# zhu-xlab/tomosar2height

Hardware: AMD Instinct MI355X
Metric: training tiles/sec (Berlin crop, cloud-only) (higher is better)
Workload: dtype f32; 1 GPU; BASELINE.json configs[1]: Berlin cloud-only, fp32 per-point GEMMs, train_step(tile) per tile, 4 tiles coalesced per forward/backward (Trainer default), N=131072 points/tile, R=256, ALTO depth 5, 512x512 target, optimize_every=64; points_per_tile=131072, optimize_every=64, train_batch=1, coalesce_tiles=4, optimizer=t2h FlatAdamW (one kernel over the flat bucket), parallelism=dp1, rccl_ranks=0, channels_last=True, point_distribution=70 % in 160 buildings + 30 % uniform, grid_convs=conv_bx3.hip: fp32 products from 3 fp16 MFMAs (2-way split, block scales), library_fallbacks=0, hip_graph=False

## Files before the change

tomosar2height_amd/csrc/conv_bx3.hip:

```cpp
#include <stdlib.h>
#include "t2h_common.h"
#include "gemm_args.h"
#include "gemm_tile.h"

namespace t2h {
namespace {

using bf16x8 = __attribute__((ext_vector_type(8))) __bf16;
using f16x8 = __attribute__((ext_vector_type(8))) _Float16;
using f16x2 = __attribute__((ext_vector_type(2))) _Float16;
using bf16x2 = __attribute__((ext_vector_type(2))) __bf16;
using f32x2 = __attribute__((ext_vector_type(2))) float;
using s16x4 = __attribute__((ext_vector_type(4))) short;
using s16x8 = __attribute__((ext_vector_type(8))) short;
typedef __attribute__((address_space(3))) void lds_void;
typedef const __attribute__((address_space(1))) void glb_void;
typedef __attribute__((address_space(3))) s16x4 lds_s16x4;

#ifndef T2H_BX3_BDIRECT
#define T2H_BX3_BDIRECT 1
#endif
constexpr int NT = 256;
constexpr int TW = 32;
constexpr int CC = 32;
// ... 502 lines not shown
                old.x = mk.x > 0.f ? old.x : 0.f; old.y = mk.y > 0.f ? old.y : 0.f;
                old.z = mk.z > 0.f ? old.z : 0.f; old.w = mk.w > 0.f ? old.w : 0.f;
            }
            v.x += bv.x; v.y += bv.y; v.z += bv.z; v.w += bv.w;
            if (UPM == 1) {
                float4 *dst = reinterpret_cast<float4 *>(p.y + q);
                if (accum) { v.x += old.x; v.y += old.y; v.z += old.z; v.w += old.w; }
                if (p.addend) { v.x += mk.x; v.y += mk.y; v.z += mk.z; v.w += mk.w; }
                *dst = v;
                continue;
            }
            if (p.mask) {
                v.x = mk.x > 0.f ? v.x : 0.f; v.y = mk.y > 0.f ? v.y : 0.f;
                v.z = mk.z > 0.f ? v.z : 0.f; v.w = mk.w > 0.f ? v.w : 0.f;
            }
            if (relu) { v.x = relu1(v.x); v.y = relu1(v.y); v.z = relu1(v.z); v.w = relu1(v.w); }
            float4 *dst = reinterpret_cast<float4 *>(ybase + q * p.ldy + col);
            if (accum) { v.x += old.x; v.y += old.y; v.z += old.z; v.w += old.w; }
            *dst = v;
        }
    }
  }
}

struct WgradArgs {
    const float *dy;
    const float *x;
    float *slab;
    float *colslab;
    int H, W, Cin, Cout;
    int n_units, units_per_split;
    int ldx;
    int lddy;
};

template <int COT, int NPL, bool UP = false, int GT = 0>
__global__ __launch_bounds__(NT, 2) void bx3_wgrad_kernel(WgradArgs p) {
    static_assert(!(UP && GT), "UP and GT are different forms");
    constexpr int NTAPS = GT ? GT : (UP ? 4 : 9);
    constexpr int WPC = 4 / COT;
    constexpr int TMAX = (NTAPS + WPC - 1) / WPC;
    constexpr int YS = COT == 1 ? 64 : 64 * COT + 64;
    constexpr int XS = 64;
    constexpr int YPLANE = 32 * YS, XHP = GT ? GT * TW : (UP ? 4 * TW : 3 * (TW + 2)), XPLANE = XHP * XS;
    constexpr int LDS_WORK = NPL * YPLANE + NPL * XPLANE;
    constexpr int LDS_BYTES = LDS_WORK >= 4 * 32 * 36 * 4 ? LDS_WORK : 4 * 32 * 36 * 4;
    constexpr bool H2 = NPL == 2;
    __shared__ __attribute__((aligned(1024))) unsigned char lds[LDS_BYTES + (H2 ? 64 : 0)];
    unsigned char *yimg = lds, *ximg = lds + NPL * YPLANE;
    float *slots = reinterpret_cast<float *>(lds + LDS_BYTES);

    const int tid = threadIdx.x, lane = tid & 63, wave = tid >> 6;
    const int split = GT ? blockIdx.z : blockIdx.x, ci0 = GT ? 0 : blockIdx.y * CC, co0 = (GT ? blockIdx.x : blockIdx.z) * (32 * COT);
    const int u_beg = split * p.units_per_split, u_end = min(p.n_units, u_beg + p.units_per_split);
    const int segs = p.W / TW;

    const int cot = wave / WPC, sub = wave % WPC;
    const int tap_lo = (NTAPS * sub + WPC - 1) / WPC, tap_hi = (NTAPS * (sub + 1) + WPC - 1) / WPC;

    constexpr int XF4 = XHP * 8, XPER = (XF4 + NT - 1) / NT;
    constexpr int YPER = COT;
    float4 xr[XPER], yr[YPER];
    auto load_unit = [&](int u) {
        const int xs = u % segs, row = u / segs;
        const int y = row & (p.H - 1), x0 = xs * TW;
#pragma unroll
        for (int f = 0; f < XPER; ++f) {
            const int idx = tid + f * NT;
            const int px = idx >> 3, c4 = idx & 7;
            const int hy = px / (TW + 2), hx = px - hy * (TW + 2);
            const int gy = y + hy - 1, gx = x0 + hx - 1;
            float4 v = make_float4(0.f, 0.f, 0.f, 0.f);
            if (GT) {
                if (idx < XF4) v = *reinterpret_cast<const float4 *>(p.x + ((size_t)u * TW + (px % TW)) * p.ldx + (px / TW) * 32 + c4 * 4);
            } else if (UP) {
                v = *reinterpret_cast<const float4 *>(p.x + ((size_t)(2 * row + (px >> 6)) * (2 * p.W) + 2 * x0 + (px & 63)) * p.ldx + ci0 + c4 * 4);
            } else if (idx < XF4 && (unsigned)gy < (unsigned)p.H && (unsigned)gx < (unsigned)p.W)
                v = *reinterpret_cast<const float4 *>(p.x + ((size_t)(row + hy - 1) * p.W + gx) * p.ldx + ci0 + c4 * 4);
            xr[f] = v;
        }
#pragma unroll
        for (int f = 0; f < YPER; ++f) {
            const int idx = tid + f * NT;
            const int px = idx / (8 * COT), c4 = idx % (8 * COT);
            yr[f] = *reinterpret_cast<const float4 *>(p.dy + ((size_t)row * p.W + x0 + px) * (GT ? p.lddy : p.Cout) + co0 + c4 * 4);
        }
    };
    float4 csum = make_float4(0.f, 0.f, 0.f, 0.f);
    const bool do_colsum = p.colslab != nullptr && (UP ? blockIdx.z == 0 : blockIdx.y == 0);
    int s_run = E_UNSET, ex_cur = 0, ey_cur = 0;
    auto publish_unit_max = [&](int parity) {
        float mx = 0.f, my = 0.f;
#pragma unroll
        for (int f = 0; f < XPER; ++f) mx = abs4max(mx, xr[f]);
#pragma unroll
        for (int f = 0; f < YPER; ++f) my = abs4max(my, yr[f]);
        mx = wave_max(mx);
        my = wave_max(my);
        if (lane == 0) { slots[(parity * 4 + wave) * 2] = mx; slots[(parity * 4 + wave) * 2 + 1] = my; }
    };
    auto store_unit = [&]() {
#pragma unroll
        for (int f = 0; f < XPER; ++f) {
            const int idx = tid + f * NT;
            if (idx < XF4) {
                const int c4 = idx & 7;
                int px = idx >> 3;
                if (UP) {
                    px = ((px >> 6) * 2 + (px & 1)) * TW + ((px & 63) >> 1);
                    if (do_colsum) { csum.x += xr[f].x; csum.y += xr[f].y; csum.z += xr[f].z; csum.w += xr[f].w; }
                }
                unsigned a1, a2, a3, b1, b2, b3;
                unsigned char *d = ximg + px * XS + c4 * 8;
                if (H2) {
                    split2h(xr[f].x, xr[f].y, ex_cur, a1, a2);
                    split2h(xr[f].z, xr[f].w, ex_cur, b1, b2);
                    *reinterpret_cast<uint2 *>(d) = make_uint2(a1, b1);
                    *reinterpret_cast<uint2 *>(d + XPLANE) = make_uint2(a2, b2);
                    continue;
                }
                split3(xr[f].x, xr[f].y, a1, a2, a3);
                split3(xr[f].z, xr[f].w, b1, b2, b3);
                *reinterpret_cast<uint2 *>(d) = make_uint2(a1, b1);
                if (NPL == 3) {
                    *reinterpret_cast<uint2 *>(d + XPLANE) = make_uint2(a2, b2);
                    *reinterpret_cast<uint2 *>(d + 2 * XPLANE) = make_uint2(a3, b3);
                }
            }
        }
#pragma unroll
        for (int f = 0; f < YPER; ++f) {
            const int idx = tid + f * NT;
            const int px = idx / (8 * COT), c4 = idx % (8 * COT);
            unsigned a1, a2, a3, b1, b2, b3;
            unsigned char *d = yimg + px * YS + c4 * 8;
            if (!UP && do_colsum) { csum.x += yr[f].x; csum.y += yr[f].y; csum.z += yr[f].z; csum.w += yr[f].w; }
            if (H2) {
                split2h(yr[f].x, yr[f].y, ey_cur, a1, a2);
                split2h(yr[f].z, yr[f].w, ey_cur, b1, b2);
                *reinterpret_cast<uint2 *>(d) = make_uint2(a1, b1);
                *reinterpret_cast<uint2 *>(d + YPLANE) = make_uint2(a2, b2);
                continue;
            }
            split3(yr[f].x, yr[f].y, a1, a2, a3);
            split3(yr[f].z, yr[f].w, b1, b2, b3);
            *reinterpret_cast<uint2 *>(d) = make_uint2(a1, b1);
            if (NPL == 3) {
                *reinterpret_cast<uint2 *>(d + YPLANE) = make_uint2(a2, b2);
                *reinterpret_cast<uint2 *>(d + 2 * YPLANE) = make_uint2(a3, b3);
            }
        }
    };

    f32x16 acc[TMAX];
#pragma unroll
    for (int t = 0; t < TMAX; ++t)
#pragma unroll
        for (int z = 0; z < 16; ++z) acc[t][z] = 0.0f;

    const int g = lane >> 4, gi = lane & 15, gq = gi >> 2, gp = gi & 3;
    const int kpix = 8 * (g >> 1) + gq;
    const int choff = (16 * (g & 1) + 4 * gp) * 2;
    auto tr8 = [&](const unsigned char *a, int row_stride) -> bf16x8 {
        const s16x4 lo = __builtin_amdgcn_ds_read_tr16_b64_v4i16((lds_s16x4 *)(a));
        const s16x4 hi = __builtin_amdgcn_ds_read_tr16_b64_v4i16((lds_s16x4 *)(a + 4 * row_stride));
        const s16x8 v = __builtin_shufflevector(lo, hi, 0, 1, 2, 3, 4, 5, 6, 7);
        return *reinterpret_cast<const bf16x8 *>(&v);
    };

    if (u_beg < u_end) load_unit(u_beg);
    if (H2) {
        if (u_beg < u_end) publish_unit_max(u_beg & 1);
        __syncthreads();
    }
    for (int u = u_beg; u < u_end; ++u) {
        if (H2) {
            const float *sl = slots + (u & 1) * 8;
            const int ex_nat = block_exponent(__float_as_uint(fmaxf(fmaxf(sl[0], sl[2]), fmaxf(sl[4], sl[6]))));
            const int ey_nat = block_exponent(__float_as_uint(fmaxf(fmaxf(sl[1], sl[3]), fmaxf(sl[5], sl[7]))));
            if (ex_nat != E_UNSET && ey_nat != E_UNSET && ex_nat + ey_nat < s_run) {
                if (s_run != E_UNSET) {
#pragma unroll
                    for (int t = 0; t < TMAX; ++t)
#pragma unroll
                        for (int z = 0; z < 16; ++z) acc[t][z] = ldexpf(acc[t][z], ex_nat + ey_nat - s_run);
                }
                s_run = ex_nat + ey_nat;
            }
            ex_cur = ex_nat == E_UNSET ? 0 : ex_nat;
            ey_cur = ey_nat == E_UNSET ? 0 : (s_run == E_UNSET ? ey_nat : min(s_run - ex_cur, ey_nat));
        }
        store_unit();
        if (u + 1 < u_end) load_unit(u + 1);
        __syncthreads();
#pragma unroll
        for (int s = 0; s < 2; ++s) {
            bf16x8 af[NPL];
            const unsigned char *ya = yimg + (16 * s + kpix) * YS + cot * 64 + choff;
#pragma unroll
            for (int pl = 0; pl < NPL; ++pl) af[pl] = tr8(ya + pl * YPLANE, YS);
#pragma unroll
            for (int t = 0; t < TMAX; ++t) {
                const int tap = tap_lo + t;
                if (tap < tap_hi) {
                    const int ky = tap / 3, kx = tap - 3 * ky;
                    const unsigned char *xa = ximg + ((UP || GT) ? tap * TW + 16 * s + kpix : ky * (TW + 2) + 16 * s + kpix + kx) * XS + choff;
                    bf16x8 bfr[NPL];
#pragma unroll
                    for (int pl = 0; pl < NPL; ++pl) bfr[pl] = tr8(xa + pl * XPLANE, XS);
                    constexpr int ia[6] = {2, 0, 1, 1, 0, 0}, ib[6] = {0, 2, 1, 0, 1, 0};
                    if (H2) {
#pragma unroll
                        for (int e = 3; e < 6; ++e)
                            acc[t] = __builtin_amdgcn_mfma_f32_32x32x16_f16(*reinterpret_cast<const f16x8 *>(&af[ia[e]]),
                                                                            *reinterpret_cast<const f16x8 *>(&bfr[ib[e]]), acc[t], 0, 0, 0);
                    } else {
#pragma unroll
                        for (int e = (NPL == 3 ? 0 : 5); e < 6; ++e)
                            acc[t] = __builtin_amdgcn_mfma_f32_32x32x16_bf16(af[ia[e]], bfr[ib[e]], acc[t], 0, 0, 0);
                    }
                }
            }
        }
        if (H2 && u + 1 < u_end) publish_unit_max((u + 1) & 1);
        __syncthreads();
    }

    if (do_colsum) {
        float4 *red = reinterpret_cast<float4 *>(lds);
        red[tid] = csum;
        __syncthreads();
        constexpr int CG = UP ? 8 : 8 * COT;
        if (tid < CG) {
            float4 tsum = red[tid];
            for (int j = tid + CG; j < NT; j += CG) { tsum.x += red[j].x; tsum.y += red[j].y; tsum.z += red[j].z; tsum.w += red[j].w; }
            if (UP) *reinterpret_cast<float4 *>(p.colslab + (size_t)split * p.Cin + ci0 + tid * 4) = tsum;
            else *reinterpret_cast<float4 *>(p.colslab + (size_t)split * p.Cout + co0 + tid * 4) = tsum;
        }
        __syncthreads();
    }

    float *patch = reinterpret_cast<float *>(lds) + wave * (32 * 36);
    const int er = lane >> 3, ec = (lane & 7) * 4, r = lane & 31, h = lane >> 5;
    float *sbase = p.slab + (size_t)split * p.Cout * NTAPS * p.Cin;
#pragma unroll
    for (int t = 0; t < TMAX; ++t) {
        const int tap = tap_lo + t;
        if (tap < tap_hi) {
#pragma unroll
            for (int z = 0; z < 16; ++z)
                patch[((z & 3) + 8 * (z >> 2) + 4 * h) * 36 + r] = H2 ? ldexpf(acc[t][z], s_run == E_UNSET ? 0 : -s_run) : acc[t][z];
#pragma unroll
            for (int pass = 0; pass < 4; ++pass) {
                const float4 v = *reinterpret_cast<const float4 *>(patch + (pass * 8 + er) * 36 + ec);
                const int co = co0 + cot * 32 + pass * 8 + er;
                *reinterpret_cast<float4 *>(sbase + ((size_t)co * NTAPS + tap) * p.Cin + ci0 + ec) = v;
            }
        }
    }
}

bool al16(const void *q) { return (uintptr_t)q % 16 == 0; }
bool pow2(int v) { return v > 0 && (v & (v - 1)) == 0; }

int check_bx3(const char *what, int B, int H, int W, int Cin, int Cout) {
    if (B < 1 || !pow2(H) || !pow2(W) || H < 4 || W < TW || H > 32768 || W > 32768 || Cin < 32 || Cout < 32 || Cin % 32 || Cout % 32)
        return fail(T2H_ERR_ARG, "%s: needs power-of-two H >= 4, W >= 32 and Cin, Cout multiples of 32 (B=%d H=%d W=%d %d->%d)", what, B,
                    H, W, Cin, Cout);
    if ((long long)B * H * W > (1LL << 30)) return fail(T2H_ERR_ARG, "%s: more than 2^30 pixels", what);
    return T2H_OK;
}

struct RowsPlan { bool tall; int bn, splits, chunks_per_split; long long tiles; };
RowsPlan bx3_rows_plan(int B, int H, int W, int Kc, int Nc, int ntap = 9, int upm = 0) {
    RowsPlan r{};
    r.bn = Nc % 128 == 0 ? 128 : (Nc % 64 == 0 ? 64 : 32);
    if (upm) {
        r.tall = false;
        const long long row_tiles = (long long)B * (H / 4) * (W / TW);
        if (upm == 1) while (r.bn > 32 && row_tiles * (Nc / r.bn) < 192) r.bn >>= 1;
        r.tiles = row_tiles * (Nc / r.bn);
        r.splits = 1;
        const int nchunk_u = Kc / 64;
        static const long long target_u = 512;
        if (upm == 2 && r.tiles < target_u / 2) {
            long long want = (target_u + r.tiles - 1) / r.tiles;
            if (want > nchunk_u) want = nchunk_u;
            if (want > 32) want = 32;
            r.splits = (int)(want < 1 ? 1 : want);
// ... 88 lines not shown
            else BX3_LAUNCH(4, 32, 4, 1, 32, 9);
        }
    } else if (ntap == 1 && upm == 0 && npl == 2 && a.Kc == 64 && r.splits == 1 && a.Nc / r.bn >= 8 && persist_n_enabled()) {
        const long long row_tiles = (long long)a.B * (a.H / 4) * (a.W / TW);
        const int pbn = r.bn == 128 ? 64 : r.bn;
        const int ntn = a.Nc / pbn;
        static const long long persist_wgs = getenv("T2H_BX3_PERSIST_WGS") ? atoll(getenv("T2H_BX3_PERSIST_WGS")) : 2048;
        static const long long min_groups = getenv("T2H_BX3_PERSIST_MIN_GROUPS") ? atoll(getenv("T2H_BX3_PERSIST_MIN_GROUPS")) : 4;
        long long groups = persist_wgs / (row_tiles > 0 ? row_tiles : 1);
        if (groups < min_groups) groups = min_groups;
        if (groups < 1) groups = 1;
        if (groups > ntn) groups = ntn;
        a.ntn_per_wg = (int)((ntn + groups - 1) / groups);
        groups = (ntn + a.ntn_per_wg - 1) / a.ntn_per_wg;
        const long long pgrid = row_tiles * groups;
        if (pbn == 64) { hipLaunchKernelGGL((bx3_rows_kernel<4, 64, 4, 1, 64, 2, 1, 0, true>), dim3((unsigned)pgrid), dim3(NT), 0, s, a); note_kernel("bx3_rows_kernel<4,64,4,1,64,2,1,0,true>"); }
        else { hipLaunchKernelGGL((bx3_rows_kernel<4, 32, 4, 1, 64, 2, 1, 0, true>), dim3((unsigned)pgrid), dim3(NT), 0, s, a); note_kernel("bx3_rows_kernel<4,32,4,1,64,2,1,0,true>"); }
    } else {
        if (r.tall) {
            if (r.bn == 128) BX3_LAUNCH(8, 128, 2, 2, 32, 1);
            else if (r.bn == 64) BX3_LAUNCH(8, 64, 4, 1, 32, 1);
            else BX3_LAUNCH(8, 32, 4, 1, 32, 1);
        } else {
            if (r.bn == 128) BX3_LAUNCH(4, 128, 2, 2, 64, 1);
            else if (r.bn == 64) BX3_LAUNCH(4, 64, 4, 1, 64, 1);
            else BX3_LAUNCH(4, 32, 4, 1, 64, 1);
        }
    }
    if (int rc = check_launch(what)) return rc;
    if (r.splits > 1) return launch_reduce_rows_epilogue(static_cast<const float *>(ws), r.splits, M * a.Nc, M, a.Nc, e, s);
    return T2H_OK;
}

struct WgradPlan { int cot, splits, units_per_split, n_units; };
WgradPlan bx3_wgrad_plan(int B, int H, int W, int Cin, int Cout) {
    WgradPlan p{};
    p.cot = Cout % 128 == 0 ? 4 : (Cout % 64 == 0 ? 2 : 1);
    p.n_units = B * H * (W / TW);
    const long long groups = (long long)(Cin / CC) * (Cout / (32 * p.cot));
    static const long long forced = getenv("T2H_BX3_WGRAD_WGS") ? atoll(getenv("T2H_BX3_WGRAD_WGS")) : 0;
    const long long target = forced > 0 ? forced : ((long long)H * W <= 128 * 128 ? 256 : 512);
    long long splits = target / groups;
    if (splits < 1) splits = 1;
    if (splits > p.n_units) splits = p.n_units;
    p.units_per_split = (int)((p.n_units + splits - 1) / splits);
    p.splits = (p.n_units + p.units_per_split - 1) / p.units_per_split;
    return p;
}

}
}

using namespace t2h;

T2H_API int t2h_conv3x3_bx3_supported(int B, int H, int W, int Cin, int Cout) {
    return B >= 1 && pow2(H) && pow2(W) && H >= 4 && W >= TW && H <= 32768 && W <= 32768 && Cin >= 32 && Cout >= 32 && Cin % 32 == 0 &&
           Cout % 32 == 0 && (long long)B * H * W <= (1LL << 30);
}

T2H_API size_t t2h_conv3x3_bx3_weights_bytes(int Cin, int Cout) {
    if (Cin < 32 || Cout < 32 || Cin % 32 || Cout % 32) return 0;
    return (size_t)Cout * 9 * Cin * 6;
}

T2H_API int t2h_conv3x3_bx3_prepare(const float *w, int Cin, int Cout, int transposed, void *wf, t2h_stream_t stream) {
    if (!w || !wf) return fail(T2H_ERR_ARG, "conv3x3_bx3_prepare: null pointer");
    if (Cin < 32 || Cout < 32 || Cin % 32 || Cout % 32 || !al16(wf))
        return fail(T2H_ERR_ARG, "conv3x3_bx3_prepare: Cin=%d, Cout=%d must be multiples of 32, wf 16-byte aligned", Cin, Cout);
    const int Kc = transposed ? Cout : Cin, Nc = transposed ? Cin : Cout;
    const long long total = (long long)(Kc / 16) * 9 * (Nc / 32) * 64;
    const unsigned blocks = (unsigned)((total + 255) / 256);
    if (transposed) hipLaunchKernelGGL(bx3_prepare_kernel<true>, dim3(blocks), dim3(256), 0, as_stream(stream), w, Cin, Cout, static_cast<unsigned *>(wf));
// ... 33 lines not shown
    if (!al16(dy) || !al16(wf_t) || !al16(dx) || (mask && !al16(mask))) return fail(T2H_ERR_ARG, "conv3x3_bx3_dgrad: pointers must be 16-byte aligned");
    RowsArgs a{};
    a.x = dy; a.wf = static_cast<const unsigned *>(wf_t); a.bias = nullptr; a.mask = mask; a.y = dx;
    a.B = B; a.H = H; a.W = W; a.Kc = Cout; a.Nc = Cin; a.ldx = Cout; a.ldy = Cin; a.ldm = Cin;
    a.flags = (flags & T2H_ACCUM) ? F_ACCUM : 0;
    a.wscale = f16_trailer(wf_t, (size_t)Cout * 9 * Cin * 4);
    return launch_rows(a, npl_of(flags), workspace, workspace_bytes, as_stream(stream), "conv3x3_bx3_dgrad");
}

T2H_API int t2h_conv3x3_bx3_dgrad_rank1_supported(int B, int H, int W, int Cin, int Cout) {
    if (!t2h_conv3x3_bx3_supported(B, H, W, Cin, Cout)) return 0;
    return bx3_rows_plan(B, H, W, Cout, Cin).splits == 1;
}

T2H_API int t2h_conv3x3_bx3_dgrad_rank1(const float *dy, const void *wf_t, float *dx, const float *mask, const float *g, const float *w1,
                                        int B, int H, int W, int Cin, int Cout, int flags, t2h_stream_t stream) {
    if (!dy || !wf_t || !dx || !g || !w1) return fail(T2H_ERR_ARG, "conv3x3_bx3_dgrad_rank1: null pointer");
    if (int rc = check_bx3("conv3x3_bx3_dgrad_rank1", B, H, W, Cin, Cout)) return rc;
    if (!t2h_conv3x3_bx3_dgrad_rank1_supported(B, H, W, Cin, Cout))
        return fail(T2H_ERR_ARG, "conv3x3_bx3_dgrad_rank1: this shape splits its reduction (use t2h_conv3x3_bx3_dgrad with T2H_ACCUM)");
    if (flags & T2H_ACCUM) return fail(T2H_ERR_ARG, "conv3x3_bx3_dgrad_rank1: the rank-1 term takes the place of the accumulated values");
    if (!al16(dy) || !al16(wf_t) || !al16(dx) || (mask && !al16(mask)) || !al16(w1))
        return fail(T2H_ERR_ARG, "conv3x3_bx3_dgrad_rank1: pointers must be 16-byte aligned");
    RowsArgs a{};
    a.x = dy; a.wf = static_cast<const unsigned *>(wf_t); a.bias = nullptr; a.mask = mask; a.y = dx;
    a.B = B; a.H = H; a.W = W; a.Kc = Cout; a.Nc = Cin; a.ldx = Cout; a.ldy = Cin; a.ldm = Cin;
    a.flags = 0; a.r1_g = g; a.r1_w = w1;
    a.wscale = f16_trailer(wf_t, (size_t)Cout * 9 * Cin * 4);
    return launch_rows(a, npl_of(flags), nullptr, 0, as_stream(stream), "conv3x3_bx3_dgrad_rank1");
}

T2H_API size_t t2h_conv3x3_bx3_wgrad_workspace_bytes(int B, int H, int W, int Cin, int Cout) {
    if (!t2h_conv3x3_bx3_supported(B, H, W, Cin, Cout)) return 0;
    WgradPlan p = bx3_wgrad_plan(B, H, W, Cin, Cout);
    return (size_t)p.splits * ((size_t)Cout * 9 * Cin + Cout) * sizeof(float);
}

T2H_API int t2h_conv3x3_bx3_wgrad(const float *dy, const float *x, float *dw, float *db, int B, int H, int W, int Cin, int Cout,
                                  int flags, void *workspace, size_t workspace_bytes, t2h_stream_t stream) {
    if (!dy || !x || !dw) return fail(T2H_ERR_ARG, "conv3x3_bx3_wgrad: null pointer");
    if (int rc = check_bx3("conv3x3_bx3_wgrad", B, H, W, Cin, Cout)) return rc;
    if (!al16(dy) || !al16(x)) return fail(T2H_ERR_ARG, "conv3x3_bx3_wgrad: pointers must be 16-byte aligned");
    const size_t need = t2h_conv3x3_bx3_wgrad_workspace_bytes(B, H, W, Cin, Cout);
    if (!workspace || workspace_bytes < need || !al16(workspace))
        return fail(T2H_ERR_WORKSPACE, "conv3x3_bx3_wgrad: workspace %zu < %zu bytes", workspace_bytes, need);
    hipStream_t s = as_stream(stream);
    WgradPlan p = bx3_wgrad_plan(B, H, W, Cin, Cout);
    const int Ncols = 9 * Cin;
    float *slab = static_cast<float *>(workspace);
    float *colslab = slab + (size_t)p.splits * Cout * Ncols;
    WgradArgs a{};
    a.dy = dy; a.x = x; a.slab = slab; a.colslab = db ? colslab : nullptr;
    a.H = H; a.W = W; a.Cin = Cin; a.Cout = Cout; a.n_units = p.n_units; a.units_per_split = p.units_per_split; a.ldx = Cin;
    dim3 grid(p.splits, Cin / CC, Cout / (32 * p.cot));
    if (grid.y > 65535 || grid.z > 65535) return fail(T2H_ERR_ARG, "conv3x3_bx3_wgrad: too many channel chunks");
    if (flags & T2H_F16X2) {
        if (p.cot == 4) { hipLaunchKernelGGL((bx3_wgrad_kernel<4, 2>), grid, dim3(NT), 0, s, a); note_kernel("bx3_wgrad_kernel<4,2,false,0>"); }
        else if (p.cot == 2) { hipLaunchKernelGGL((bx3_wgrad_kernel<2, 2>), grid, dim3(NT), 0, s, a); note_kernel("bx3_wgrad_kernel<2,2,false,0>"); }
        else { hipLaunchKernelGGL((bx3_wgrad_kernel<1, 2>), grid, dim3(NT), 0, s, a); note_kernel("bx3_wgrad_kernel<1,2,false,0>"); }
    } else if (flags & T2H_BF16) {
        if (p.cot == 4) { hipLaunchKernelGGL((bx3_wgrad_kernel<4, 1>), grid, dim3(NT), 0, s, a); note_kernel("bx3_wgrad_kernel<4,1,false,0>"); }
        else if (p.cot == 2) { hipLaunchKernelGGL((bx3_wgrad_kernel<2, 1>), grid, dim3(NT), 0, s, a); note_kernel("bx3_wgrad_kernel<2,1,false,0>"); }
        else { hipLaunchKernelGGL((bx3_wgrad_kernel<1, 1>), grid, dim3(NT), 0, s, a); note_kernel("bx3_wgrad_kernel<1,1,false,0>"); }
    } else {
        if (p.cot == 4) { hipLaunchKernelGGL((bx3_wgrad_kernel<4, 3>), grid, dim3(NT), 0, s, a); note_kernel("bx3_wgrad_kernel<4,3,false,0>"); }
        else if (p.cot == 2) { hipLaunchKernelGGL((bx3_wgrad_kernel<2, 3>), grid, dim3(NT), 0, s, a); note_kernel("bx3_wgrad_kernel<2,3,false,0>"); }
        else { hipLaunchKernelGGL((bx3_wgrad_kernel<1, 3>), grid, dim3(NT), 0, s, a); note_kernel("bx3_wgrad_kernel<1,3,false,0>"); }
    }
    if (int rc = check_launch("conv3x3_bx3_wgrad")) return rc;
    return launch_reduce_slabs(slab, p.splits, (long long)Cout * Ncols, Cout, Ncols, Ncols, (flags & T2H_ACCUM) ? 1 : 0, dw, colslab, db, s,
                               0, 0, (flags & T2H_DEFER_REDUCE) != 0);
}

T2H_API int t2h_gemm_bx3_supported(int64_t M, int K, int N) {
    return M >= 128 && M % 128 == 0 && M <= (1LL << 30) && K >= 64 && K % 64 == 0 && N >= 32 && N % 32 == 0;
}

T2H_API size_t t2h_gemm_bx3_weights_bytes(int K, int N) {
    if (K < 16 || N < 32 || K % 16 || N % 32) return 0;
    return (size_t)K * N * 6;
}

T2H_API int t2h_gemm_bx3_prepare(const float *w, int ldw, int K, int N, int w_is_kn, void *wf, t2h_stream_t stream) {
    if (!w || !wf) return fail(T2H_ERR_ARG, "gemm_bx3_prepare: null pointer");
    if (K < 16 || N < 32 || K % 16 || N % 32 || !al16(wf) || ldw < (w_is_kn ? N : K))
        return fail(T2H_ERR_ARG, "gemm_bx3_prepare: K=%d must be a multiple of 16, N=%d of 32, ldw=%d at least the row length", K, N, ldw);
    const long long total = (long long)(K / 16) * (N / 32) * 64;
// ... 32 lines not shown
    if (splits > units) splits = units;
    if (splits < 1) splits = 1;
    const long long per = (units + splits - 1) / splits;
    return (int)((units + per - 1) / per);
}

T2H_API int t2h_gemm_bx3_wgrad_supported(int64_t M, int K, int N) {
    return M >= TW && M % TW == 0 && M <= (1LL << 30) && (K == 64 || K == 128 || K == 256) && N >= 64 && N % 64 == 0;
}

T2H_API size_t t2h_gemm_bx3_wgrad_workspace_bytes(int64_t M, int K, int N) {
    if (!t2h_gemm_bx3_wgrad_supported(M, K, N)) return 0;
    return (size_t)gemm_wgrad_splits(M, N) * ((size_t)N * K + N) * sizeof(float);
}

T2H_API int t2h_gemm_bx3_wgrad(const float *dy, int lddy, const float *x, int ldx, int64_t M, int K, int N, float *dw, float *db, int flags,
                               void *workspace, size_t workspace_bytes, t2h_stream_t stream) {
    if (!dy || !x || !dw) return fail(T2H_ERR_ARG, "gemm_bx3_wgrad: null pointer");
    if (!t2h_gemm_bx3_wgrad_supported(M, K, N))
        return fail(T2H_ERR_ARG, "gemm_bx3_wgrad: needs M %% 32 == 0, K in {64, 128, 256}, N %% 64 == 0 (M=%lld K=%d N=%d)", (long long)M, K, N);
    if (lddy < N || ldx < K || lddy % 4 || ldx % 4 || !al16(dy) || !al16(x))
        return fail(T2H_ERR_ARG, "gemm_bx3_wgrad: rows must be 16-byte aligned and at least N / K floats long");
    if (!(flags & T2H_F16X2)) return fail(T2H_ERR_ARG, "gemm_bx3_wgrad: only the fp16 two-way split (T2H_F16X2) is built");
    const size_t need = t2h_gemm_bx3_wgrad_workspace_bytes(M, K, N);
    if (!workspace || workspace_bytes < need || !al16(workspace))
        return fail(T2H_ERR_WORKSPACE, "gemm_bx3_wgrad: workspace %zu < %zu bytes", workspace_bytes, need);
    hipStream_t s = as_stream(stream);
    const int splits = gemm_wgrad_splits(M, N);
    float *slab = static_cast<float *>(workspace);
    float *colslab = slab + (size_t)splits * N * K;
    WgradArgs a{};
    a.dy = dy; a.x = x; a.slab = slab; a.colslab = db ? colslab : nullptr;
    a.H = (int)(M / TW); a.W = TW; a.Cin = 32; a.Cout = N; a.n_units = (int)(M / TW);
    a.units_per_split = (a.n_units + splits - 1) / splits; a.ldx = ldx; a.lddy = lddy;
    const dim3 grid(N / 64, 1, splits);
    if (grid.z > 65535) return fail(T2H_ERR_ARG, "gemm_bx3_wgrad: too many splits");
    if (K == 64) { hipLaunchKernelGGL((bx3_wgrad_kernel<2, 2, false, 2>), grid, dim3(NT), 0, s, a); note_kernel("bx3_wgrad_kernel<2,2,false,2>"); }
    else if (K == 128) { hipLaunchKernelGGL((bx3_wgrad_kernel<2, 2, false, 4>), grid, dim3(NT), 0, s, a); note_kernel("bx3_wgrad_kernel<2,2,false,4>"); }
    else { hipLaunchKernelGGL((bx3_wgrad_kernel<2, 2, false, 8>), grid, dim3(NT), 0, s, a); note_kernel("bx3_wgrad_kernel<2,2,false,8>"); }
    if (int rc = check_launch("gemm_bx3_wgrad")) return rc;
    return launch_reduce_slabs(slab, splits, (long long)N * K, N, K, K, (flags & T2H_ACCUM) ? 1 : 0, dw, colslab, db, s, 0, 0,
                               (flags & T2H_DEFER_REDUCE) != 0);
}

static int check_up_bx3(const char *what, int B, int H, int W, int Cin, int Cout) {
    if (B < 1 || !pow2(H) || !pow2(W) || H > 16384 || W > 16384 || (long long)B * H * W % 128 != 0 || (long long)B * H * W > (1LL << 28) ||
        Cin < 64 || Cout < 64 || Cin % 64 || Cout % 64)
        return fail(T2H_ERR_ARG, "%s: needs power-of-two H, W with B H W %% 128 == 0 and Cin, Cout multiples of 64 (B=%d H=%d W=%d %d->%d)",
                    what, B, H, W, Cin, Cout);
    return T2H_OK;
}
static int ilog2i(int v) { int l = 0; while ((1 << l) < v) ++l; return l; }

T2H_API int t2h_upconv2x2_bx3_supported(int B, int H, int W, int Cin, int Cout) {
    return B >= 1 && pow2(H) && pow2(W) && H <= 16384 && W <= 16384 && (long long)B * H * W % 128 == 0 && (long long)B * H * W <= (1LL << 28) &&
           Cin >= 64 && Cout >= 64 && Cin % 64 == 0 && Cout % 64 == 0;
}

T2H_API int t2h_upconv2x2_bx3_fwd(const float *x, const void *wf, const float *bias, const float *addend, float *y, int B, int H, int W,
                                  int Cin, int Cout, int flags, t2h_stream_t stream) {
    if (!x || !wf || !y) return fail(T2H_ERR_ARG, "upconv2x2_bx3_fwd: null pointer");
    if (int rc = check_up_bx3("upconv2x2_bx3_fwd", B, H, W, Cin, Cout)) return rc;
    if (!al16(x) || !al16(wf) || !al16(y) || (bias && !al16(bias)) || (addend && !al16(addend)))
        return fail(T2H_ERR_ARG, "upconv2x2_bx3_fwd: pointers must be 16-byte aligned");
    const long long M = (long long)B * H * W;
    RowsArgs a{};
    a.x = x; a.wf = static_cast<const unsigned *>(wf); a.bias = bias; a.addend = addend; a.y = y;
// ... 35 lines not shown
    static const long long forced = getenv("T2H_BX3_UPWGRAD_WGS") ? atoll(getenv("T2H_BX3_UPWGRAD_WGS")) : 0;
    long long splits = (forced > 0 ? forced : 256) / groups;
    if (splits < 1) splits = 1;
    if (splits > p.n_units) splits = p.n_units;
    p.units_per_split = (int)((p.n_units + splits - 1) / splits);
    p.splits = (p.n_units + p.units_per_split - 1) / p.units_per_split;
    return p;
}

T2H_API size_t t2h_upconv2x2_bx3_wgrad_workspace_bytes(int B, int H, int W, int Cin, int Cout) {
    if (!t2h_upconv2x2_bx3_supported(B, H, W, Cin, Cout) || W < TW) return 0;
    const WgradPlan p = up_wgrad_plan(B, H, W, Cin, Cout);
    return (size_t)p.splits * ((size_t)Cin * 4 * Cout + Cout) * sizeof(float);
}

T2H_API int t2h_upconv2x2_bx3_wgrad(const float *dy, int lddy, const float *x, float *dw, float *db, int B, int H, int W, int Cin,
                                    int Cout, int flags, void *workspace, size_t workspace_bytes, t2h_stream_t stream) {
    if (!dy || !x || !dw) return fail(T2H_ERR_ARG, "upconv2x2_bx3_wgrad: null pointer");
    if (int rc = check_up_bx3("upconv2x2_bx3_wgrad", B, H, W, Cin, Cout)) return rc;
    if (lddy < Cout || lddy % 4) return fail(T2H_ERR_ARG, "upconv2x2_bx3_wgrad: lddy=%d must be >= Cout=%d and a multiple of 4", lddy, Cout);
    if (W < TW) return fail(T2H_ERR_ARG, "upconv2x2_bx3_wgrad: W=%d below the %d-pixel unit", W, TW);
    if (!al16(dy) || !al16(x)) return fail(T2H_ERR_ARG, "upconv2x2_bx3_wgrad: pointers must be 16-byte aligned");
    const size_t need = t2h_upconv2x2_bx3_wgrad_workspace_bytes(B, H, W, Cin, Cout);
    if (!workspace || workspace_bytes < need || !al16(workspace))
        return fail(T2H_ERR_WORKSPACE, "upconv2x2_bx3_wgrad: workspace %zu < %zu bytes", workspace_bytes, need);
    hipStream_t s = as_stream(stream);
    const WgradPlan p = up_wgrad_plan(B, H, W, Cin, Cout);
    const int Ncols = 4 * Cout;
    float *slab = static_cast<float *>(workspace);
    float *colslab = slab + (size_t)p.splits * Cin * Ncols;
    WgradArgs a{};
    a.dy = x; a.x = dy; a.slab = slab; a.colslab = db ? colslab : nullptr;
    a.H = H; a.W = W; a.Cin = Cout; a.Cout = Cin; a.n_units = p.n_units; a.units_per_split = p.units_per_split; a.ldx = lddy;
    dim3 grid(p.splits, Cout / CC, Cin / (32 * p.cot));
    if (grid.y > 65535 || grid.z > 65535) return fail(T2H_ERR_ARG, "upconv2x2_bx3_wgrad: too many channel chunks");
    if (flags & T2H_F16X2) {
        if (p.cot == 4) { hipLaunchKernelGGL((bx3_wgrad_kernel<4, 2, true>), grid, dim3(NT), 0, s, a); note_kernel("bx3_wgrad_kernel<4,2,true,0>"); }
        else { hipLaunchKernelGGL((bx3_wgrad_kernel<2, 2, true>), grid, dim3(NT), 0, s, a); note_kernel("bx3_wgrad_kernel<2,2,true,0>"); }
    } else if (p.cot == 4) { hipLaunchKernelGGL((bx3_wgrad_kernel<4, 3, true>), grid, dim3(NT), 0, s, a); note_kernel("bx3_wgrad_kernel<4,3,true,0>"); }
    else { hipLaunchKernelGGL((bx3_wgrad_kernel<2, 3, true>), grid, dim3(NT), 0, s, a); note_kernel("bx3_wgrad_kernel<2,3,true,0>"); }
    if (int rc = check_launch("upconv2x2_bx3_wgrad")) return rc;
    return launch_reduce_slabs(slab, p.splits, (long long)Cin * Ncols, Cin, Ncols, Ncols, (flags & T2H_ACCUM) ? 1 : 0, dw, colslab, db, s,
                               p.splits, Cout, (flags & T2H_DEFER_REDUCE) != 0);
}

T2H_API size_t t2h_conv3x3_f16x2_weights_bytes(int Cin, int Cout) {
    if (Cin < 32 || Cout < 32 || Cin % 32 || Cout % 32) return 0;
    return (size_t)Cout * 9 * Cin * 4 + 256;
}

static int absmax_into(const float *w, long long rows, int cols, long long ld, unsigned *trailer, hipStream_t s, const char *what) {
    if (hipMemsetAsync(trailer, 0, 256, s) != hipSuccess) return fail(T2H_ERR_LAUNCH, "%s: hipMemsetAsync failed", what);
    const long long total = rows * cols;
    const unsigned blocks = (unsigned)std::min<long long>((total + 4095) / 4096, 1024);
    hipLaunchKernelGGL(absmax_kernel, dim3(blocks ? blocks : 1), dim3(256), 0, s, w, rows, cols, ld, trailer);
    return check_launch(what);
}

T2H_API int t2h_conv3x3_f16x2_prepare(const float *w, int Cin, int Cout, int transposed, void *wf, t2h_stream_t stream) {
    if (!w || !wf) return fail(T2H_ERR_ARG, "conv3x3_f16x2_prepare: null pointer");
    if (Cin < 32 || Cout < 32 || Cin % 32 || Cout % 32 || !al16(wf))
        return fail(T2H_ERR_ARG, "conv3x3_f16x2_prepare: Cin=%d, Cout=%d must be multiples of 32, wf 16-byte aligned", Cin, Cout);
    hipStream_t s = as_stream(stream);
    unsigned *trailer = reinterpret_cast<unsigned *>(static_cast<unsigned char *>(wf) + (size_t)Cout * 9 * Cin * 4);
    if (int rc = absmax_into(w, 1, Cout * 9 * Cin, 0, trailer, s, "conv3x3_f16x2_prepare")) return rc;
    const int Kc = transposed ? Cout : Cin, Nc = transposed ? Cin : Cout;
// ... 53 lines not shown
```

Baseline: 194.8 tiles/s.

## Tile conv3x3 wgrad over two input-channel chunks and two-row units

The 3x3 weight-gradient kernel now lets one workgroup cover up to two 32-channel input chunks (waves split across chunks) and process units of two image rows, sharing the halo rows and the dy tile across them. Per-chunk block-exponent tracking is added for the fp16x2 path, and the plan halves the unit count and shrinks the grid's channel dimension. This is meant to cut redundant dy loads and halo re-reads and the per-unit sync overhead, in exchange for more registers and LDS per workgroup and fewer tap slices per wave, which may hurt occupancy or balance.

After: 196.2 tiles/s, median of 6. Within noise of the previous version (+0.7%).

```diff
diff --git a/tomosar2height_amd/csrc/conv_bx3.hip b/tomosar2height_amd/csrc/conv_bx3.hip
--- a/tomosar2height_amd/csrc/conv_bx3.hip
+++ b/tomosar2height_amd/csrc/conv_bx3.hip
@@ -558,99 +558,142 @@
     int n_units, units_per_split;
     int ldx;
     int lddy;
+    int cit;
 };
+
+constexpr int wgrad_ys(int cot) { return cot == 1 ? 64 : 64 * cot + 64; }
+constexpr bool wgrad_fits(int cot, int npl, int cit, int ur) {
+    const int wpp = 4 / (cot * cit), tmax = (9 + wpp - 1) / wpp;
+    const int xf4 = ((ur + 2) * (TW + 2) * 8 + NT - 1) / NT;
+    return 16 * tmax + 4 * (ur * cot + cit * xf4) <= 176 &&
+           npl * (ur * TW * wgrad_ys(cot) + cit * (ur + 2) * (TW + 2) * 64) <= 65536 - 128;
+}
+constexpr int wgrad_citmax(int cot, int npl) { return cot <= 2 && (wgrad_fits(cot, npl, 2, 2) || wgrad_fits(cot, npl, 2, 1)) ? 2 : 1; }
+constexpr int wgrad_unit_rows(int cot, int npl) { return wgrad_fits(cot, npl, wgrad_citmax(cot, npl), 2) ? 2 : 1; }
 
 template <int COT, int NPL, bool UP = false, int GT = 0>
 __global__ __launch_bounds__(NT, 2) void bx3_wgrad_kernel(WgradArgs p) {
     static_assert(!(UP && GT), "UP and GT are different forms");
+    constexpr bool PLAIN = !UP && !GT;
     constexpr int NTAPS = GT ? GT : (UP ? 4 : 9);
-    constexpr int WPC = 4 / COT;
-    constexpr int TMAX = (NTAPS + WPC - 1) / WPC;
-    constexpr int YS = COT == 1 ? 64 : 64 * COT + 64;
+    constexpr int CITMAX = PLAIN ? wgrad_citmax(COT, NPL) : 1;
+    constexpr int UR = PLAIN ? wgrad_unit_rows(COT, NPL) : 1;
+    constexpr int SUB = PLAIN ? 2 / UR : 1;
+    constexpr int WPPMIN = 4 / (COT * CITMAX);
+    constexpr int TMAX = (NTAPS + WPPMIN - 1) / WPPMIN;
+    constexpr int YS = wgrad_ys(COT);
     constexpr int XS = 64;
-    constexpr int YPLANE = 32 * YS, XHP = GT ? GT * TW : (UP ? 4 * TW : 3 * (TW + 2)), XPLANE = XHP * XS;
+    constexpr int YPX = UR * TW;
+    constexpr int XHP = GT ? GT * TW : (UP ? 4 * TW : (UR + 2) * (TW + 2));
+    constexpr int YPLANE = YPX * YS, XCH = XHP * XS, XPLANE = CITMAX * XCH;
     constexpr int LDS_WORK = NPL * YPLANE + NPL * XPLANE;
     constexpr int LDS_BYTES = LDS_WORK >= 4 * 32 * 36 * 4 ? LDS_WORK : 4 * 32 * 36 * 4;
     constexpr bool H2 = NPL == 2;
-    __shared__ __attribute__((aligned(1024))) unsigned char lds[LDS_BYTES + (H2 ? 64 : 0)];
+    constexpr int SW = CITMAX + 1;
+    static_assert(LDS_BYTES + 128 <= 65536, "wgrad images exceed a workgroup's LDS");
+    __shared__ __attribute__((aligned(1024))) unsigned char lds[LDS_BYTES + (H2 ? 128 : 0)];
     unsigned char *yimg = lds, *ximg = lds + NPL * YPLANE;
     float *slots = reinterpret_cast<float *>(lds + LDS_BYTES);
 
     const int tid = threadIdx.x, lane = tid & 63, wave = tid >> 6;
-    const int split = GT ? blockIdx.z : blockIdx.x, ci0 = GT ? 0 : blockIdx.y * CC, co0 = (GT ? blockIdx.x : blockIdx.z) * (32 * COT);
-    const int u_beg = split * p.units_per_split, u_end = min(p.n_units, u_beg + p.units_per_split);
+    const int cit = CITMAX > 1 ? p.cit : 1;
+    const int split = GT ? blockIdx.z : blockIdx.x, ci0 = GT ? 0 : blockIdx.y * CC * cit, co0 = (GT ? blockIdx.x : blockIdx.z) * (32 * COT);
+    const int v_beg = split * p.units_per_split * SUB, v_end = min(p.n_units, (split + 1) * p.units_per_split) * SUB;
     const int segs = p.W / TW;
 
-    const int cot = wave / WPC, sub = wave % WPC;
-    const int tap_lo = (NTAPS * sub + WPC - 1) / WPC, tap_hi = (NTAPS * (sub + 1) + WPC - 1) / WPC;
+    const int wpp = 4 / (COT * cit);
+    const int pair = wave / wpp, sub = wave % wpp;
+    const int cot = pair / cit, cix = pair % cit;
+    const int tap_lo = (NTAPS * sub + wpp - 1) / wpp, tap_hi = (NTAPS * (sub + 1) + wpp - 1) / wpp;
 
     constexpr int XF4 = XHP * 8, XPER = (XF4 + NT - 1) / NT;
-    constexpr int YPER = COT;
-    float4 xr[XPER], yr[YPER];
-    auto load_unit = [&](int u) {
-        const int xs = u % segs, row = u / segs;
+    constexpr int YPER = UR * COT;
+    float4 xr[CITMAX][XPER], yr[YPER];
+    auto load_unit = [&](int v) {
+        int xs, row;
+        if (PLAIN) { const int pu = v / SUB; xs = pu % segs; row = (pu / segs) * 2 + (v % SUB) * UR; }
+        else { xs = v % segs; row = v / segs; }
         const int y = row & (p.H - 1), x0 = xs * TW;
 #pragma unroll
-        for (int f = 0; f < XPER; ++f) {
-            const int idx = tid + f * NT;
-            const int px = idx >> 3, c4 = idx & 7;
-            const int hy = px / (TW + 2), hx = px - hy * (TW + 2);
-            const int gy = y + hy - 1, gx = x0 + hx - 1;
-            float4 v = make_float4(0.f, 0.f, 0.f, 0.f);
-            if (GT) {
-                if (idx < XF4) v = *reinterpret_cast<const float4 *>(p.x + ((size_t)u * TW + (px % TW)) * p.ldx + (px / TW) * 32 + c4 * 4);
-            } else if (UP) {
-                v = *reinterpret_cast<const float4 *>(p.x + ((size_t)(2 * row + (px >> 6)) * (2 * p.W) + 2 * x0 + (px & 63)) * p.ldx + ci0 + c4 * 4);
-            } else if (idx < XF4 && (unsigned)gy < (unsigned)p.H && (unsigned)gx < (unsigned)p.W)
-                v = *reinterpret_cast<const float4 *>(p.x + ((size_t)(row + hy - 1) * p.W + gx) * p.ldx + ci0 + c4 * 4);
-            xr[f] = v;
+        for (int c = 0; c < CITMAX; ++c) {
+            if (c < cit) {
+#pragma unroll
+                for (int f = 0; f < XPER; ++f) {
+                    const int idx = tid + f * NT;
+                    const int px = idx >> 3, c4 = idx & 7;
+                    const int hy = px / (TW + 2), hx = px - hy * (TW + 2);
+                    const int gy = y + hy - 1, gx = x0 + hx - 1;
+                    float4 v4 = make_float4(0.f, 0.f, 0.f, 0.f);
+                    if (GT) {
+                        if (idx < XF4) v4 = *reinterpret_cast<const float4 *>(p.x + ((size_t)v * TW + (px % TW)) * p.ldx + (px / TW) * 32 + c4 * 4);
+                    } else if (UP) {
+                        v4 = *reinterpret_cast<const float4 *>(p.x + ((size_t)(2 * row + (px >> 6)) * (2 * p.W) + 2 * x0 + (px & 63)) * p.ldx + ci0 + c4 * 4);
+                    } else if (idx < XF4 && (unsigned)gy < (unsigned)p.H && (unsigned)gx < (unsigned)p.W)
+                        v4 = *reinterpret_cast<const float4 *>(p.x + ((size_t)(row + hy - 1) * p.W + gx) * p.ldx + ci0 + c * CC + c4 * 4);
+                    xr[c][f] = v4;
+                }
+            }
         }
 #pragma unroll
         for (int f = 0; f < YPER; ++f) {
             const int idx = tid + f * NT;
             const int px = idx / (8 * COT), c4 = idx % (8 * COT);
-            yr[f] = *reinterpret_cast<const float4 *>(p.dy + ((size_t)row * p.W + x0 + px) * (GT ? p.lddy : p.Cout) + co0 + c4 * 4);
+            yr[f] = *reinterpret_cast<const float4 *>(p.dy + ((size_t)(row + (px >> 5)) * p.W + x0 + (px & 31)) * (GT ? p.lddy : p.Cout) + co0 + c4 * 4);
         }
     };
     float4 csum = make_float4(0.f, 0.f, 0.f, 0.f);
     const bool do_colsum = p.colslab != nullptr && (UP ? blockIdx.z == 0 : blockIdx.y == 0);
-    int s_run = E_UNSET, ex_cur = 0, ey_cur = 0;
+    int s_run[CITMAX], ex_cur[CITMAX], ey_cur = 0;
+#pragma unroll
+    for (int c = 0; c < CITMAX; ++c) { s_run[c] = E_UNSET; ex_cur[c] = 0; }
     auto publish_unit_max = [&](int parity) {
-        float mx = 0.f, my = 0.f;
-#pragma unroll
-        for (int f = 0; f < XPER; ++f) mx = abs4max(mx, xr[f]);
+        float my = 0.f;
 #pragma unroll
         for (int f = 0; f < YPER; ++f) my = abs4max(my, yr[f]);
-        mx = wave_max(mx);
         my = wave_max(my);
-        if (lane == 0) { slots[(parity * 4 + wave) * 2] = mx; slots[(parity * 4 + wave) * 2 + 1] = my; }
+        if (lane == 0) slots[(parity * 4 + wave) * SW + CITMAX] = my;
+#pragma unroll
+        for (int c = 0; c < CITMAX; ++c) {
+            if (c < cit) {
+                float mx = 0.f;
+#pragma unroll
+                for (int f = 0; f < XPER; ++f) mx = abs4max(mx, xr[c][f]);
+                mx = wave_max(mx);
+                if (lane == 0) slots[(parity * 4 + wave) * SW + c] = mx;
+            }
+        }
     };
     auto store_unit = [&]() {
 #pragma unroll
-        for (int f = 0; f < XPER; ++f) {
-            const int idx = tid + f * NT;
-            if (idx < XF4) {
-                const int c4 = idx & 7;
-                int px = idx >> 3;
-                if (UP) {
-                    px = ((px >> 6) * 2 + (px & 1)) * TW + ((px & 63) >> 1);
-                    if (do_colsum) { csum.x += xr[f].x; csum.y += xr[f].y; csum.z += xr[f].z; csum.w += xr[f].w; }
-                }
-                unsigned a1, a2, a3, b1, b2, b3;
-                unsigned char *d = ximg + px * XS + c4 * 8;
-                if (H2) {
-                    split2h(xr[f].x, xr[f].y, ex_cur, a1, a2);
-                    split2h(xr[f].z, xr[f].w, ex_cur, b1, b2);
-                    *reinterpret_cast<uint2 *>(d) = make_uint2(a1, b1);
-                    *reinterpret_cast<uint2 *>(d + XPLANE) = make_uint2(a2, b2);
-                    continue;
-                }
-                split3(xr[f].x, xr[f].y, a1, a2, a3);
-                split3(xr[f].z, xr[f].w, b1, b2, b3);
-                *reinterpret_cast<uint2 *>(d) = make_uint2(a1, b1);
-                if (NPL == 3) {
-                    *reinterpret_cast<uint2 *>(d + XPLANE) = make_uint2(a2, b2);
-                    *reinterpret_cast<uint2 *>(d + 2 * XPLANE) = make_uint2(a3, b3);
+        for (int c = 0; c < CITMAX; ++c) {
+            if (c < cit) {
+#pragma unroll
+                for (int f = 0; f < XPER; ++f) {
+                    const int idx = tid + f * NT;
+                    if (idx < XF4) {
+                        const int c4 = idx & 7;
+                        int px = idx >> 3;
+                        if (UP) {
+                            px = ((px >> 6) * 2 + (px & 1)) * TW + ((px & 63) >> 1);
+                            if (do_colsum) { csum.x += xr[c][f].x; csum.y += xr[c][f].y; csum.z += xr[c][f].z; csum.w += xr[c][f].w; }
+                        }
+                        unsigned a1, a2, a3, b1, b2, b3;
+                        unsigned char *d = ximg + c * XCH + px * XS + c4 * 8;
+                        if (H2) {
+                            split2h(xr[c][f].x, xr[c][f].y, ex_cur[c], a1, a2);
+                            split2h(xr[c][f].z, xr[c][f].w, ex_cur[c], b1, b2);
+                            *reinterpret_cast<uint2 *>(d) = make_uint2(a1, b1);
+                            *reinterpret_cast<uint2 *>(d + XPLANE) = make_uint2(a2, b2);
+                            continue;
+                        }
+                        split3(xr[c][f].x, xr[c][f].y, a1, a2, a3);
+                        split3(xr[c][f].z, xr[c][f].w, b1, b2, b3);
+                        *reinterpret_cast<uint2 *>(d) = make_uint2(a1, b1);
+                        if (NPL == 3) {
+                            *reinterpret_cast<uint2 *>(d + XPLANE) = make_uint2(a2, b2);
+                            *reinterpret_cast<uint2 *>(d + 2 * XPLANE) = make_uint2(a3, b3);
+                        }
+                    }
                 }
             }
         }
@@ -694,33 +737,41 @@
         return *reinterpret_cast<const bf16x8 *>(&v);
     };
 
-    if (u_beg < u_end) load_unit(u_beg);
+    if (v_beg < v_end) load_unit(v_beg);
     if (H2) {
-        if (u_beg < u_end) publish_unit_max(u_beg & 1);
+        if (v_beg < v_end) publish_unit_max(v_beg & 1);
         __syncthreads();
     }
-    for (int u = u_beg; u < u_end; ++u) {
+    for (int v = v_beg; v < v_end; ++v) {
         if (H2) {
-            const float *sl = slots + (u & 1) * 8;
-            const int ex_nat = block_exponent(__float_as_uint(fmaxf(fmaxf(sl[0], sl[2]), fmaxf(sl[4], sl[6]))));
-            const int ey_nat = block_exponent(__float_as_uint(fmaxf(fmaxf(sl[1], sl[3]), fmaxf(sl[5], sl[7]))));
-            if (ex_nat != E_UNSET && ey_nat != E_UNSET && ex_nat + ey_nat < s_run) {
-                if (s_run != E_UNSET) {
-#pragma unroll
-                    for (int t = 0; t < TMAX; ++t)
-#pragma unroll
-                        for (int z = 0; z < 16; ++z) acc[t][z] = ldexpf(acc[t][z], ex_nat + ey_nat - s_run);
+            const float *sl = slots + (v & 1) * 4 * SW;
+            auto smax = [&](int k) { return __float_as_uint(fmaxf(fmaxf(sl[k], sl[SW + k]), fmaxf(sl[2 * SW + k], sl[3 * SW + k]))); };
+            const int ey_nat = block_exponent(smax(CITMAX));
+            ey_cur = ey_nat == E_UNSET ? 0 : ey_nat;
+            int rescale = 0;
+#pragma unroll
+            for (int c = 0; c < CITMAX; ++c) {
+                if (c < cit) {
+                    const int ex_nat = block_exponent(smax(c));
+                    if (ex_nat != E_UNSET && ey_nat != E_UNSET && ex_nat + ey_nat < s_run[c]) {
+                        if (s_run[c] != E_UNSET && c == cix) rescale = ex_nat + ey_nat - s_run[c];
+                        s_run[c] = ex_nat + ey_nat;
+                    }
+                    ex_cur[c] = ex_nat == E_UNSET ? 0 : (s_run[c] == E_UNSET ? ex_nat : min(s_run[c] - ey_cur, ex_nat));
                 }
-                s_run = ex_nat + ey_nat;
-            }
-            ex_cur = ex_nat == E_UNSET ? 0 : ex_nat;
-            ey_cur = ey_nat == E_UNSET ? 0 : (s_run == E_UNSET ? ey_nat : min(s_run - ex_cur, ey_nat));
+            }
+            if (rescale != 0) {
+#pragma unroll
+                for (int t = 0; t < TMAX; ++t)
+#pragma unroll
+                    for (int z = 0; z < 16; ++z) acc[t][z] = ldexpf(acc[t][z], rescale);
+            }
         }
         store_unit();
-        if (u + 1 < u_end) load_unit(u + 1);
+        if (v + 1 < v_end) load_unit(v + 1);
         __syncthreads();
-#pragma unroll
-        for (int s = 0; s < 2; ++s) {
+#pragma unroll(UR == 1 ? 2 : 1)
+        for (int s = 0; s < 2 * UR; ++s) {
             bf16x8 af[NPL];
             const unsigned char *ya = yimg + (16 * s + kpix) * YS + cot * 64 + choff;
 #pragma unroll
@@ -730,7 +781,8 @@
                 const int tap = tap_lo + t;
                 if (tap < tap_hi) {
                     const int ky = tap / 3, kx = tap - 3 * ky;
-                    const unsigned char *xa = ximg + ((UP || GT) ? tap * TW + 16 * s + kpix : ky * (TW + 2) + 16 * s + kpix + kx) * XS + choff;
+                    const unsigned char *xa = ximg + cix * XCH +
+                        ((UP || GT) ? tap * TW + 16 * s + kpix : ((s >> 1) + ky) * (TW + 2) + 16 * (s & 1) + kpix + kx) * XS + choff;
                     bf16x8 bfr[NPL];
 #pragma unroll
                     for (int pl = 0; pl < NPL; ++pl) bfr[pl] = tr8(xa + pl * XPLANE, XS);
@@ -748,7 +800,7 @@
                 }
             }
         }
-        if (H2 && u + 1 < u_end) publish_unit_max((u + 1) & 1);
+        if (H2 && v + 1 < v_end) publish_unit_max((v + 1) & 1);
         __syncthreads();
     }
 
@@ -766,6 +818,9 @@
         __syncthreads();
     }
 
+    int s_mine = s_run[0];
+#pragma unroll
+    for (int c = 1; c < CITMAX; ++c) s_mine = c == cix ? s_run[c] : s_mine;
     float *patch = reinterpret_cast<float *>(lds) + wave * (32 * 36);
     const int er = lane >> 3, ec = (lane & 7) * 4, r = lane & 31, h = lane >> 5;
     float *sbase = p.slab + (size_t)split * p.Cout * NTAPS * p.Cin;
@@ -775,12 +830,12 @@
         if (tap < tap_hi) {
 #pragma unroll
             for (int z = 0; z < 16; ++z)
-                patch[((z & 3) + 8 * (z >> 2) + 4 * h) * 36 + r] = H2 ? ldexpf(acc[t][z], s_run == E_UNSET ? 0 : -s_run) : acc[t][z];
+                patch[((z & 3) + 8 * (z >> 2) + 4 * h) * 36 + r] = H2 ? ldexpf(acc[t][z], s_mine == E_UNSET ? 0 : -s_mine) : acc[t][z];
 #pragma unroll
             for (int pass = 0; pass < 4; ++pass) {
-                const float4 v = *reinterpret_cast<const float4 *>(patch + (pass * 8 + er) * 36 + ec);
+                const float4 v4 = *reinterpret_cast<const float4 *>(patch + (pass * 8 + er) * 36 + ec);
                 const int co = co0 + cot * 32 + pass * 8 + er;
-                *reinterpret_cast<float4 *>(sbase + ((size_t)co * NTAPS + tap) * p.Cin + ci0 + ec) = v;
+                *reinterpret_cast<float4 *>(sbase + ((size_t)co * NTAPS + tap) * p.Cin + ci0 + cix * CC + ec) = v4;
             }
         }
     }
@@ -935,12 +990,14 @@
     return T2H_OK;
 }
 
-struct WgradPlan { int cot, splits, units_per_split, n_units; };
-WgradPlan bx3_wgrad_plan(int B, int H, int W, int Cin, int Cout) {
+struct WgradPlan { int cot, cit, splits, units_per_split, n_units; };
+WgradPlan bx3_wgrad_plan(int B, int H, int W, int Cin, int Cout, int npl) {
     WgradPlan p{};
     p.cot = Cout % 128 == 0 ? 4 : (Cout % 64 == 0 ? 2 : 1);
-    p.n_units = B * H * (W / TW);
-    const long long groups = (long long)(Cin / CC) * (Cout / (32 * p.cot));
+    const int citmax = npl == 2 ? wgrad_citmax(p.cot, 2) : (npl == 1 ? wgrad_citmax(p.cot, 1) : wgrad_citmax(p.cot, 3));
+    p.cit = (Cin / CC) % citmax == 0 ? citmax : 1;
+    p.n_units = B * (H / 2) * (W / TW);
+    const long long groups = (long long)(Cin / (CC * p.cit)) * (Cout / (32 * p.cot));
     static const long long forced = getenv("T2H_BX3_WGRAD_WGS") ? atoll(getenv("T2H_BX3_WGRAD_WGS")) : 0;
     const long long target = forced > 0 ? forced : ((long long)H * W <= 128 * 128 ? 256 : 512);
     long long splits = target / groups;
@@ -1040,8 +1097,9 @@
 
 T2H_API size_t t2h_conv3x3_bx3_wgrad_workspace_bytes(int B, int H, int W, int Cin, int Cout) {
     if (!t2h_conv3x3_bx3_supported(B, H, W, Cin, Cout)) return 0;
-    WgradPlan p = bx3_wgrad_plan(B, H, W, Cin, Cout);
-    return (size_t)p.splits * ((size_t)Cout * 9 * Cin + Cout) * sizeof(float);
+    int splits = 0;
+    for (int npl = 1; npl <= 3; ++npl) splits = std::max(splits, bx3_wgrad_plan(B, H, W, Cin, Cout, npl).splits);
+    return (size_t)splits * ((size_t)Cout * 9 * Cin + Cout) * sizeof(float);
 }
 
 T2H_API int t2h_conv3x3_bx3_wgrad(const float *dy, const float *x, float *dw, float *db, int B, int H, int W, int Cin, int Cout,
@@ -1053,14 +1111,15 @@
     if (!workspace || workspace_bytes < need || !al16(workspace))
         return fail(T2H_ERR_WORKSPACE, "conv3x3_bx3_wgrad: workspace %zu < %zu bytes", workspace_bytes, need);
     hipStream_t s = as_stream(stream);
-    WgradPlan p = bx3_wgrad_plan(B, H, W, Cin, Cout);
+    WgradPlan p = bx3_wgrad_plan(B, H, W, Cin, Cout, npl_of(flags));
     const int Ncols = 9 * Cin;
     float *slab = static_cast<float *>(workspace);
     float *colslab = slab + (size_t)p.splits * Cout * Ncols;
     WgradArgs a{};
     a.dy = dy; a.x = x; a.slab = slab; a.colslab = db ? colslab : nullptr;
     a.H = H; a.W = W; a.Cin = Cin; a.Cout = Cout; a.n_units = p.n_units; a.units_per_split = p.units_per_split; a.ldx = Cin;
-    dim3 grid(p.splits, Cin / CC, Cout / (32 * p.cot));
+    a.cit = p.cit;
+    dim3 grid(p.splits, Cin / (CC * p.cit), Cout / (32 * p.cot));
     if (grid.y > 65535 || grid.z > 65535) return fail(T2H_ERR_ARG, "conv3x3_bx3_wgrad: too many channel chunks");
     if (flags & T2H_F16X2) {
         if (p.cot == 4) { hipLaunchKernelGGL((bx3_wgrad_kernel<4, 2>), grid, dim3(NT), 0, s, a); note_kernel("bx3_wgrad_kernel<4,2,false,0>"); }
@@ -1159,7 +1218,7 @@
     WgradArgs a{};
     a.dy = dy; a.x = x; a.slab = slab; a.colslab = db ? colslab : nullptr;
     a.H = (int)(M / TW); a.W = TW; a.Cin = 32; a.Cout = N; a.n_units = (int)(M / TW);
-    a.units_per_split = (a.n_units + splits - 1) / splits; a.ldx = ldx; a.lddy = lddy;
+    a.units_per_split = (a.n_units + splits - 1) / splits; a.ldx = ldx; a.lddy = lddy; a.cit = 1;
     const dim3 grid(N / 64, 1, splits);
     if (grid.z > 65535) return fail(T2H_ERR_ARG, "gemm_bx3_wgrad: too many splits");
     if (K == 64) { hipLaunchKernelGGL((bx3_wgrad_kernel<2, 2, false, 2>), grid, dim3(NT), 0, s, a); note_kernel("bx3_wgrad_kernel<2,2,false,2>"); }
@@ -1261,6 +1320,7 @@
     WgradArgs a{};
     a.dy = x; a.x = dy; a.slab = slab; a.colslab = db ? colslab : nullptr;
     a.H = H; a.W = W; a.Cin = Cout; a.Cout = Cin; a.n_units = p.n_units; a.units_per_split = p.units_per_split; a.ldx = lddy;
+    a.cit = 1;
     dim3 grid(p.splits, Cout / CC, Cin / (32 * p.cot));
     if (grid.y > 65535 || grid.z > 65535) return fail(T2H_ERR_ARG, "upconv2x2_bx3_wgrad: too many channel chunks");
     if (flags & T2H_F16X2) {
```
